# dnbaker/dashing

Hardware: AMD Instinct MI355X
Metric: genome-pairs/sec, all-pairs HLL Jaccard (Ertl-MLE), N=10000 p=14 (higher is better)
Workload: dtype u8/u32 popcount + f64 estimator; 1 GPU; BASELINE configs[2]: 10000 synthetic sketches, p=14 (16384 B each), all-pairs dist on MI355X; n_sketches=10000, p=14, k=31, estimator=ERTL_MLE

## Files before the change

### dashing_amd/csrc/abi.hip

```cpp
#include <algorithm>
#include <cstdlib>
#include <cstring>
#include <new>

#include "ctx.h"

using namespace dsh;

extern "C" {

const char *dsh_backend_name(void) { return "hip:gfx950"; }

int dsh_abi_version(void) { return DSH_ABI_VERSION; }

int dsh_device_count(void)
{
    int n = 0;
    if (hipGetDeviceCount(&n) != hipSuccess) return 0;
    return n;
}

static void release_ctx(dsh_ctx *c)
{
    (void)hipSetDevice(c->device);
// ... 529 lines not shown
        *out = 0;
#endif
    }
    else if (!std::strcmp(name, "npad")) *out = c->lay.Npad;
    else if (!std::strcmp(name, "kpad")) *out = c->Kpad;
    else if (!std::strcmp(name, "cum_bytes")) *out = c->cum_bytes;
    else if (!std::strcmp(name, "sorted")) *out = c->lay.sorted;
    else if (!std::strcmp(name, "ncols")) *out = (int64_t)c->lay.ncols;
    else if (!std::strcmp(name, "lockstep")) *out = c->planes_valid && use_lockstep(c) ? 1 : 0;
    else if (!std::strcmp(name, "tiles")) *out = (int64_t)c->pp.T.size();
    else if (!std::strcmp(name, "bands")) *out = (int64_t)c->last_bands;
    else if (!std::strcmp(name, "items")) *out = (int64_t)c->pp.items.size();
    else if (!std::strcmp(name, "frag_items")) {
        uint64_t f = 0;
        for (uint32_t x : c->pp.band_frags) f += x;
        *out = (int64_t)f;
    }
    else if (!std::strcmp(name, "sparse_items")) *out = (int64_t)c->pp.sp_items.size();
    else if (!std::strcmp(name, "sparse_plane_us")) *out = (int64_t)(c->sparse_ms * 1000.0);
    else if (!std::strcmp(name, "sparse_sided_items")) *out = (int64_t)c->pp.sided_items;
    else if (!std::strcmp(name, "sparse_transposed_items")) *out = (int64_t)c->pp.transposed_items;
    else if (!std::strcmp(name, "sparse_slabs")) *out = (int64_t)c->pp.slabs.size();
    else if (!std::strcmp(name, "sparse_table_slabs")) *out = (int64_t)c->pp.table_slabs;
    else if (!std::strcmp(name, "sparse_planes")) *out = c->sparse_planes;
    else if (!std::strcmp(name, "sparse_sided")) *out = c->sparse_sided;
    else if (!std::strcmp(name, "sparse_cap")) *out = c->sparse_cap;
    else if (!std::strcmp(name, "words_per_plane")) *out = c->W;
    else if (!std::strcmp(name, "avg_tile_planes_x100")) {
        uint64_t tot = 0;
        for (const auto &t : c->pp.T) tot += t.w - t.z;
        *out = c->pp.T.empty() ? 0 : (int64_t)(tot * 100 / c->pp.T.size());
    }
    else return fail(c, DSH_EINVAL, "unknown info %s", name);
    return DSH_OK;
}

}

struct IntOption {
    const char *name;
    int64_t lo, hi;
    const char *range;
    void (*set)(dsh_ctx *c, int64_t v);
};
#define OPT_TO(member, T) [](dsh_ctx *c, int64_t v) { c->member = (T)v; }
static_assert(kGreedyMaxRows == 8192 && plan::kSparseCapMax == 2040, "the ranges below name these");
static const IntOption kIntOptions[] = {
    {"cum_budget_bytes", 1 << 20, INT64_MAX, "too small", OPT_TO(cum_budget, uint64_t)},
    {"knn_square_budget_bytes", 0, INT64_MAX, "must be >= 0", OPT_TO(knn_square_budget, uint64_t)},
    {"threshold_band_bytes", 4, INT64_MAX, "must be at least 4", OPT_TO(threshold_band_bytes, uint64_t)},
    {"pairs_chunk", 1, 1 << 24, "must be in [1, 2^24]", OPT_TO(pairs.chunk, uint64_t)},
    {"cluster_chunk", 1, 1 << 26, "must be in [1, 2^26]", OPT_TO(cc.chunk, uint64_t)},
    {"stats_route", -1, 1, "must be -1 (auto), 0 (dense) or 1 (pairs)", OPT_TO(gs.route, int)},
    {"linkage_route", -1, 1, "must be -1 (auto), 0 (dense) or 1 (pairs)", OPT_TO(lk.route, int)},
    {"linkage_partition", 0, 1, "must be 0 or 1", OPT_TO(lk.partition, int)},
    {"linkage_budget_bytes", 64, INT64_MAX, "must be at least 64", OPT_TO(lk.budget, uint64_t)},
    {"linkage_lds_max", 0, 6144, "must be in [0, 6144]", OPT_TO(lk.lds_max, uint32_t)},
    {"greedy_band_rows", 1, kGreedyMaxRows, "must be in [1, 8192]", OPT_TO(gr.band_rows, uint64_t)},
    {"derive_chunk_bytes", 1, INT64_MAX, "must be at least 1", OPT_TO(derive.chunk_bytes, uint64_t)},
    {"curve_segment", 0, INT64_MAX, "must be >= 0 (0 = the planner's)", OPT_TO(curve.segment, uint64_t)},
    {"curve_scratch_bytes", 1, INT64_MAX, "must be at least 1", OPT_TO(curve.scratch_bytes, uint64_t)},
    {"sort", -1, 1, "must be -1, 0 or 1", OPT_TO(sort_mode, int)},
    {"nsplit", 0, 64, "must be in [0,64]", OPT_TO(nsplit, int)},
    {"part_band_tiles", 1, 1 << 30, "out of range", OPT_TO(part_band_tiles, int)},
    {"xch_tail_bands", 0, 8, "out of range", OPT_TO(tail_bands, int)},
    {"overflow_frag_permille", 0, 1000, "out of range", OPT_TO(overflow_frag_permille, int)},
    {"sparse_planes", -1, 2, "is -1 (auto), 0 (off), 1 or 2", OPT_TO(sparse_planes, int)},
    {"sparse_sided", -1, 1, "is -1 (auto), 0 (off) or 1 (forced)", OPT_TO(sparse_sided, int)},
    {"sparse_lds", 0, 1, "must be 0 or 1", OPT_TO(sparse_lds, int)},
    {"sparse_cap", 0, plan::kSparseCapMax, "must be in [0, 2040]", OPT_TO(sparse_cap, int)},
    {"xch_recv_gate", -1, 1, "is -1 (auto), 0 or 1", OPT_TO(xch.recv_gate, int)},
    {"finalize_signal", -1, 1, "is -1 (auto), 0 or 1", OPT_TO(finalize_signal, int)},
};
#undef OPT_TO

extern "C" int dsh_set_option(dsh_ctx *c, const char *name, int64_t v)
{
    if (!c || !name) return DSH_EINVAL;
    for (const IntOption &o : kIntOptions) {
        if (std::strcmp(name, o.name)) continue;
        if (v < o.lo || v > o.hi) return fail(c, DSH_EINVAL, "%s %s", o.name, o.range);
        o.set(c, v);
        return DSH_OK;
    }
    if (!std::strcmp(name, "kc")) {
        if (v != 0 && v != 16 && v != 32) return fail(c, DSH_EINVAL, "kc must be 0 (auto), 16 or 32");
        c->kc_opt = (int)v;
        c->planes_valid = false;
        return DSH_OK;
    }
    if (!std::strcmp(name, "pair_groups")) {
        if (v != 0 && v != 2 && v != 3) return fail(c, DSH_EINVAL, "pair_groups must be 0 (auto), 2 or 3");
// ... 34 lines not shown
```

### dashing_amd/csrc/ctx.h

```cpp
#pragma once
#include <hip/hip_runtime.h>
#include <rccl/rccl.h>

#include <cstdarg>
#include <cstdio>
#include <cstdlib>
#include <deque>
#include <string>
#include <vector>

#include "../../include/dashing_hip.h"
#include "kernels.h"
#include "plan.h"

struct NoCopy {
    NoCopy() = default;
    NoCopy(const NoCopy &) = delete;
    NoCopy &operator=(const NoCopy &) = delete;
};

struct DevBuf : NoCopy {
    void *ptr = nullptr;
    size_t cap = 0;
    ~DevBuf() { release(); }
// ... 146 lines not shown
    const uint32_t *hk32 = nullptr;
    const uint32_t *hg32 = nullptr;
    const uint32_t *hv32 = nullptr;
    uint32_t pass_sparse_cap = 0;
    bool hk32_valid = false;
    double host_layout_us = 0, host_lists_us = 0, host_keys_wait_us = 0;
    Staging st_perm;
    DevBuf rowoff;
    Staging st_lists;
    uint32_t W = 0, Kpad = 0;
    int emax = 0, elow = 0, cum_bytes = 4;
    int kc = 16;
    int kc_opt = 0;
    int pair_groups = 3;
    int pair_groups_opt = 0;
    int emax_opt = -1;
    int elow_opt = -1;
    int part_band_tiles = 2048;
    int overflow_frag_permille = 500;
    int sparse_planes = -1;
    int sparse_cap = (int)dsh::plan::kSparseCapDefault;
    int sparse_sided = -1;
    int sparse_lds = 1;
    DevBuf sp_tab, sp_lists, sp_len, sp_slabs, sp_items;
    Staging st_sparse;
    std::vector<dsh::plan::U2> sp_have;
    uint64_t sp_serial = 0, lay_serial = 0;
    uint32_t sp_cap_have = 0;
    double sparse_ms = 0;
    std::vector<std::pair<hipEvent_t, hipEvent_t>> ev_sparse;
    int tail_bands = 2;
    std::vector<double> part_ready_ms;
    std::vector<uint64_t> part_floats;
    size_t last_bands = 0;
    uint64_t cum_budget = 8ull << 30;
    int sort_mode = -1;
    int range_sort_min_rows = 1024;
    DevBuf thr_vals;
    uint64_t threshold_band_bytes = (uint64_t)1 << 30;
    uint64_t knn_square_budget = (uint64_t)96 << 30;
    int pair_mfma = 0;
    int finalize_stop = 0;
    int finalize_timing = 0;
    DevBuf phase_cyc;
    int nsplit = 0;
    bool profiling = false;
// ... 258 lines not shown
```

### dashing_amd/csrc/engine.hip

```cpp
#include <algorithm>
#include <chrono>
#include <cstring>

#include "ctx.h"

namespace dsh {

int prepare(dsh_ctx *c, int estim, int want_sorted, bool card_only, uint64_t want_rb, uint64_t want_re, uint32_t nparts,
            int rowsorted, const std::vector<uint64_t> *extra_in)
{
    static const std::vector<uint64_t> kNoExtra;
    std::vector<uint64_t> extra_cached;
    const std::vector<uint64_t> *extra = extra_in ? extra_in : &kNoExtra;
    if (!c->have_sketches) return fail(c, DSH_ESTATE, "no sketches loaded");
    if (estim < 0 || estim > 2) return fail(c, DSH_EINVAL, "bad estimator %d", estim);
    if (want_sorted < 0) {
        want_sorted = c->lay.sorted;
        want_rb = c->lay.rb;
        want_re = c->lay.re;
        rowsorted = 0;
        extra_cached = c->lay.extra;
        extra = &extra_cached;
    }
    if (!want_sorted) rowsorted = 0, extra = &kNoExtra;
// ... 201 lines not shown
{
    JobLayout jl;
    const uint64_t jre = std::min<uint64_t>(job.row_end, c->n);
    const bool full_tri = !job.rect && job.row_begin == 0 && jre >= c->n;
    jl.with_parts = job.nparts > 0 && !job.rect && !job.sorted_rows;
    jl.lre = c->n;
    if (job.sorted_rows) jl.want_sorted = 1;
    else if (!job.rect && jre > job.row_begin &&
             (jl.with_parts || (c->sort_mode != 0 && (full_tri || jre - job.row_begin >= (uint64_t)c->range_sort_min_rows)))) {
        jl.want_sorted = 1;
        jl.lrb = job.row_begin;
        jl.lre = jre;
    }
    jl.with_extra = jl.want_sorted && jl.with_parts && !job.extra.empty() && jl.lre > jl.lrb;
    return jl;
}

constexpr uint64_t kSparseSlabBudget = 2ull << 30;
uint32_t sparse_list_stride(const dsh_ctx *c)
{
    return std::max<uint32_t>(8, (std::min<uint32_t>((uint32_t)c->sparse_cap, plan::kSparseCapMax) + 7) / 8 * 8);
}
int sparse_wordmajor(const dsh_ctx *c) { return c->sparse_lds && c->p <= 15 ? 1 : 0; }
uint64_t sparse_slab_bytes(const dsh_ctx *c)
{
    return ((uint64_t)16 << c->p) + (uint64_t)kTile * sparse_list_stride(c) * sizeof(uint16_t) + kTile * sizeof(uint32_t);
}

plan::Tuning tuning_of(const dsh_ctx *c)
{
    plan::Tuning tu;
    tu.W = c->W;
    tu.kc = c->kc;
    tu.cum_bytes = c->cum_bytes;
    tu.cum_budget = c->cum_budget;
    tu.nsplit = c->nsplit;
    tu.lockstep = use_lockstep(c);
    tu.round_items = 256u * (uint32_t)c->pair_groups;
    tu.small_round_items = c->pair_groups_opt == 0 && c->pair_groups == 3 ? 512u : 0u;
    tu.part_band_tiles = (uint32_t)c->part_band_tiles;
    tu.overflow_frag_max_permille = (uint32_t)c->overflow_frag_permille;
    tu.tail_bands = (uint32_t)c->tail_bands;
    tu.p = c->p;
    tu.sparse_planes = c->sparse_planes;
    tu.sparse_cap = (uint32_t)c->sparse_cap;
    tu.sparse_sided = c->sparse_sided;
// ... 131 lines not shown
        HIPCHK(c, launch_upload(c->stream, c->sp_slabs.ptr, h + ib, sb));
        HIPCHK(c, c->sp_tab.ensure(ns * m * 16));
        HIPCHK(c, c->sp_lists.ensure(ns * kTile * (size_t)cap * sizeof(uint16_t)));
        HIPCHK(c, c->sp_len.ensure(ns * kTile * sizeof(uint32_t)));
        HIPCHK(c, launch_sparse_build(c->stream, (const uint32_t *)c->planes.ptr, L.Npad, c->W, L.ncols, (const uint2 *)c->sp_slabs.ptr,
                                      (uint32_t)ns, cap, sparse_wordmajor(c), (uint32_t *)c->sp_tab.ptr, (uint16_t *)c->sp_lists.ptr, (uint32_t *)c->sp_len.ptr));
        c->sp_have = pp.slabs;
        c->sp_serial = c->lay_serial;
        c->sp_cap_have = cap | (uint32_t)sparse_wordmajor(c) << 31;
        timer.stop(c->prep_ms, true);
    }
    HIPCHK(c, c->st_sparse.sent(c->stream));
    return DSH_OK;
}

int launch_sparse_items(dsh_ctx *c, size_t bi, uint64_t nslots)
{
    const plan::PairPlan &pp = c->pp;
    if (bi >= pp.band_sp_items.size()) return DSH_OK;
    const auto &rg = pp.band_sp_items[bi];
    if (rg.first == rg.second) return DSH_OK;
    hipEvent_t a = c->profiling ? next_event(c) : nullptr, b = c->profiling ? next_event(c) : nullptr;
    if (a && b) (void)hipEventRecord(a, c->stream);
    HIPCHK(c, launch_sparse_count(c->stream, c->cum_bytes, (const uint4 *)c->sp_items.ptr + rg.first, (uint32_t)(rg.second - rg.first),
                                  sparse_wordmajor(c), (const uint32_t *)c->sp_tab.ptr, (const uint16_t *)c->sp_lists.ptr, (const uint32_t *)c->sp_len.ptr,
                                  sparse_list_stride(c), 1u << c->p, c->cum.ptr, nslots));
    if (a && b) {
        (void)hipEventRecord(b, c->stream);
        c->ev_sparse.emplace_back(a, b);
    }
    return DSH_OK;
}

int launch_tile_kernel(dsh_ctx *c, const PairRun &r, size_t bi, uint64_t nslots)
{
    const plan::Layout &L = c->lay;
    const plan::PairPlan &pp = c->pp;
    const uint4 *dt = (const uint4 *)c->tiles.ptr + pp.bands[bi].first;
    const uint4 *di = (const uint4 *)c->items.ptr + r.item_off[bi];
    const uint32_t ni = (uint32_t)(r.item_off[bi + 1] - r.item_off[bi]);
    if (c->pair_mfma)
        HIPCHK(c, launch_pair_counts_mfma(c->stream, c->kc, c->cum_bytes, (const uint32_t *)c->planes.ptr,
                                          L.Npad, c->Kpad, c->W, L.P, dt, di, ni, c->cum.ptr, nslots));
    else if (use_lockstep(c))
        HIPCHK(c, launch_pair_counts_lockstep(c->stream, c->kc, (int)(pp.band_round[bi] / 256), c->cum_bytes, (const uint32_t *)c->planes.ptr,
                                              L.Npad, c->Kpad, c->W, L.P, dt, di, ni, bi < pp.band_frags.size() ? pp.band_frags[bi] : 0u,
                                              c->cum.ptr, nslots));
    else
// ... 131 lines not shown
    q.col_begin = job.col_begin;
    q.col_end = job.col_end;
    r.tu = tuning_of(c);
    if (!plan::build_tiles(c->lay, q, r.tu, pp)) {
        pp.T.clear();
        return DSH_OK;
    }
    c->last_bands = pp.bands.size();
    if ((rc = reserve_lists(c, r))) return rc;
    c->host_lists_us = std::chrono::duration<double, std::micro>(std::chrono::steady_clock::now() - t_l0).count();

    if (jl.with_parts && pp.nparts >= 1 && pp.nparts <= kSigMaxParts && !c->finalize_timing && !c->finalize_stop && c->finalize_signal != 0) {
        r.signal = device_can_wait_value(c);
        if (!r.signal && c->finalize_signal == 1) return fail(c, DSH_ENODEV, "option finalize_signal = 1, but the device does not support hipStreamWaitValue32");
    }
    c->parts_signalled = r.signal;
    if (r.signal && (rc = stage_signal_block(c, r))) return rc;
    if (c->finalize_timing) {
        HIPCHK(c, c->phase_cyc.ensure(16 * sizeof(unsigned long long)));
        HIPCHK(c, hipMemsetAsync(c->phase_cyc.ptr, 0, 16 * sizeof(unsigned long long), c->stream));
    }
    r.fin = finalize_invariants(c, job, jl.with_extra);
    c->ev_sparse.clear();
    if (!pp.sp_items.empty() && (rc = prepare_sparse(c))) return rc;
    for (size_t bi = 0; bi < pp.bands.size(); ++bi) {
        const uint64_t nslots = (uint64_t)(pp.bands[bi].second - pp.bands[bi].first) * kTile * kTile;
        if ((rc = upload_band(c, r, bi))) return rc;
        hipEvent_t a = nullptr, b = nullptr, d = nullptr;
        if (c->profiling) {
            a = next_event(c);
            b = next_event(c);
            d = next_event(c);
            if (a) (void)hipEventRecord(a, c->stream);
        }
        if ((rc = launch_sparse_items(c, bi, nslots))) return rc;
        if ((rc = launch_tile_kernel(c, r, bi, nslots))) return rc;
        if (b) (void)hipEventRecord(b, c->stream);
        if (bi == 0) {
            HIPCHK(c, c->ev_first_tiles.ensure());
            HIPCHK(c, hipEventRecord(c->ev_first_tiles, c->stream));
        }
        r.fin.a.nslots = nslots;
        if ((rc = finalize_band(c, r, bi))) return rc;
        if (d) (void)hipEventRecord(d, c->stream);
        if (a && b && d) {
            r.evp.emplace_back(a, b);
// ... 9 lines not shown
```

### dashing_amd/csrc/host/plan_capi.cpp

```cpp
#include <algorithm>
#include <cstdarg>
#include <cstdio>
#include <cstring>
#include <vector>

#include "../linkage.h"
#include "../mst.h"
#include "../plan.h"
#include "../sketch_plan.h"
#include "../uf.h"

using namespace dsh;
using namespace dsh::plan;

namespace {

struct SparseCheck {
    const uint32_t *gcnt = nullptr;
    int planes = 0;
    uint32_t cap = 0;
    uint32_t *routes = nullptr;
    uint64_t routes_cap = 0;
    const uint32_t *thr = nullptr;
    uint32_t thr_cap = 0;
// ... 725 lines not shown
    sc.planes = sparse_planes;
    sc.cap = sparse_cap;
    sc.thr = thr;
    sc.thr_cap = thr_cap;
    sc.sided = sparse_sided;
    CheckJob job = base_job(n, keys, mode, want_sorted, rb, re, nparts, want_parts, p, cum_budget);
    job.cb = cb, job.ce = ce;
    job.lockstep = lockstep, job.nsplit = nsplit, job.ls_item_chunks = ls_item_chunks;
    job.extra.assign(extra, extra + (extra ? n_extra : 0));
    job.round_items = round_items;
    job.sc = &sc;
    job.resolve();
    if (!job.extra.empty() && !(job.want_sorted && job.mode == 0)) return E.fail("extra segments need a sorted triangle layout");
    Layout L;
    job_layout(job, L);
    Tuning tu;
    PairQuery q;
    PairPlan pp;
    const bool any = job_plan(job, L, tu, q, pp);
    *features = digest_plan(L, tu, q, pp, any, digests);
    return (int)kDigestSections;
}

uint64_t dshh_rowsorted_split(uint64_t n, uint64_t rb, uint64_t re) { return rowsorted_split(n, rb, re); }

int64_t dshh_threshold_bands(uint64_t n, uint64_t rb, uint64_t re, uint64_t ncols, uint64_t band_bytes, uint64_t row_cap,
                             uint64_t *bounds, uint64_t cap)
{
    const uint64_t band_floats = std::max<uint64_t>(band_bytes / sizeof(float), 1);
    if (!ncols && re > n) re = n;
    uint64_t nb = 0;
    if (cap) bounds[0] = rb;
    for (uint64_t b0 = rb; b0 < re;) {
        b0 = ncols ? std::min<uint64_t>(re, b0 + rect_band_rows(ncols, band_floats)) : tri_band_end(n, b0, re, band_floats, row_cap);
        if (++nb >= cap) return -1;
        bounds[nb] = b0;
    }
    return (int64_t)nb;
}

uint64_t dshh_hist_grid(uint64_t units, uint64_t lds_bytes, uint32_t cus, uint64_t *iters)
{
    const uint64_t grid = hist_grid(units, lds_bytes, cus);
    if (iters) *iters = units / (4 * grid) + (units % (4 * grid) ? 1 : 0);
    return grid;
}
// ... 192 lines not shown
```

### dashing_amd/csrc/kernels.h

```cpp
#pragma once
#include <hip/hip_runtime.h>
#include <stdint.h>

#include "consts.h"
#include "sketch_plan.h"

namespace dsh {

hipError_t launch_selfhist_card(hipStream_t st, const uint8_t *regs, uint64_t first, uint64_t n, int p, int estim,
                                int emax, int elow, uint32_t *hist, void *exc, uint8_t *excv, uint32_t *exc_n,
                                uint32_t *keys, uint8_t *tailhist, uint32_t *gcnt, uint32_t *sthr, uint32_t scap);
hipError_t launch_card_from_hist(hipStream_t st, const uint32_t *hist, const uint32_t *keys, uint64_t first, uint64_t n, int p,
                                 int estim, double *card);
inline int colindex_inline(int p, uint32_t E) { return p <= 12 && E <= 256 ? 7 : 3; }
struct ColIndexLaunch {
    const void *exc;
    const uint8_t *excv;
    const uint32_t *exc_n, *keys;
    const double *card;
    const uint8_t *tailhist;
    const uint32_t *perm;
    uint64_t ncols;
    int p;
    uint32_t nblocks, nbuckets, ent_stride, E;
    uint32_t *rec;
    uint32_t *ent;
    uint32_t *nS, *keyS;
    double *cardS;
    uint8_t *thS;
    uint32_t *rl;
};
hipError_t launch_build_colindex(hipStream_t st, const ColIndexLaunch &c);
hipError_t launch_transform(hipStream_t st, const uint8_t *regs, uint64_t n, int p, int vlo,
                            uint32_t P, uint32_t W, uint32_t Npad, uint32_t *planes,
                            const uint32_t *perm);
hipError_t launch_pair_counts(hipStream_t st, int kc, int cum_bytes, const uint32_t *planes,
                              uint32_t Npad, uint32_t Kpad, uint32_t W, uint32_t P,
                              const uint4 *tiles, const uint4 *items, uint32_t nitems, void *cum,
                              uint64_t nslots);

hipError_t launch_sparse_build(hipStream_t st, const uint32_t *planes, uint32_t Npad, uint32_t W, uint64_t ncols, const uint2 *slabs,
                               uint32_t nslabs, uint32_t cap, int wordmajor, uint32_t *tab, uint16_t *lists, uint32_t *len);
hipError_t launch_sparse_count(hipStream_t st, int cum_bytes, const uint4 *items, uint32_t nitems, int wordmajor, const uint32_t *tab,
                               const uint16_t *lists, const uint32_t *len, uint32_t cap, uint32_t m, void *cum, uint64_t nslots);

hipError_t launch_pair_counts_lockstep(hipStream_t st, int kc, int groups, int cum_bytes, const uint32_t *planes,
                                       uint32_t Npad, uint32_t Kpad, uint32_t W, uint32_t P, const uint4 *tiles,
                                       const uint4 *items, uint32_t nitems, uint32_t nfrag, void *cum, uint64_t nslots);
hipError_t launch_pair_counts_mfma(hipStream_t st, int kc, int cum_bytes, const uint32_t *planes,
                                   uint32_t Npad, uint32_t Kpad, uint32_t W, uint32_t P,
                                   const uint4 *tiles, const uint4 *items, uint32_t nitems, void *cum,
                                   uint64_t nslots);

struct FinalizeArgs {
    const void *cum;
    uint64_t nslots;
    const uint4 *tiles;
    const uint32_t *perm;
    const uint64_t *rowoff;
    int hist_bins;
    int pbase;
    int p;
    int estim;
    int result_type;
    double ksinv;
    const uint32_t *nS;
    const uint32_t *keyS;
// ... 219 lines not shown
```

### dashing_amd/csrc/kernels_sparseplane.hip

```cpp
#include <hip/hip_runtime.h>
#include <stdint.h>

#include <algorithm>

#include "kernels.h"
#include "plan.h"

namespace dsh {

namespace {

using plan::kSpItemListA;
using plan::kSpItemTabA;
using plan::kSpItemTransposed;
using plan::kSpPlaneMask;
using plan::kSpSlabA;
using plan::kSpSlabTableOnly;

constexpr int kSpChunk = 16;
constexpr int kSpCounters = 11;

__global__ __launch_bounds__(256) void k_sparse_build(const uint32_t *__restrict__ planes, uint32_t Npad, uint32_t W, uint64_t ncols,
                                                      const uint2 *__restrict__ slabs, uint32_t nslabs, uint32_t cap, int wordmajor,
                                                      uint32_t *__restrict__ tab, uint16_t *__restrict__ lists, uint32_t *__restrict__ len)
{
    const uint32_t lane = threadIdx.x & 63u;
// ... 46 lines not shown
    }
}

__device__ __forceinline__ void csa(uint32_t &h, uint32_t &l, uint32_t a, uint32_t b, uint32_t c)
{
    const uint32_t u = a ^ b;
    h = (a & b) | (u & c);
    l = u ^ c;
}

__device__ __forceinline__ void put32(uint16_t *dst, const uint32_t (&v)[32])
{
#pragma unroll
    for (int q = 0; q < 4; ++q)
        reinterpret_cast<uint4 *>(dst)[q] = make_uint4(v[8 * q] | (v[8 * q + 1] << 16), v[8 * q + 2] | (v[8 * q + 3] << 16),
                                                       v[8 * q + 4] | (v[8 * q + 5] << 16), v[8 * q + 6] | (v[8 * q + 7] << 16));
}
__device__ __forceinline__ void put32(uint32_t *dst, const uint32_t (&v)[32])
{
#pragma unroll
    for (int q = 0; q < 8; ++q) reinterpret_cast<uint4 *>(dst)[q] = make_uint4(v[4 * q], v[4 * q + 1], v[4 * q + 2], v[4 * q + 3]);
}

template <typename CT>
__device__ __forceinline__ void sp_values(uint32_t (&out)[32], const uint32_t (&c)[kSpCounters], uint32_t fl, uint32_t m, uint32_t ll,
                                          const uint32_t *lt)
{
    const bool la = (fl & kSpItemListA) != 0, ta = (fl & kSpItemTabA) != 0;
    const uint32_t kl = !la && !ta ? m - ll : la && !ta ? ll : 0u;
    const uint32_t tsub = !la && !ta ? 0xFFFFFFFFu : 0u, tadd = !la && ta ? 0xFFFFFFFFu : 0u;
    const uint32_t cneg = la != ta ? 0xFFFFFFFFu : 0u;
#pragma unroll
    for (int cc = 0; cc < 32; ++cc) {
        uint32_t cnt = 0;
#pragma unroll
        for (int b = 0; b < kSpCounters; ++b) cnt |= ((c[b] >> cc) & 1u) << b;
        const uint32_t t = lt[cc];
        out[cc] = (kl + (t & tadd) - (t & tsub) + ((cnt ^ cneg) - cneg)) & (sizeof(CT) == 2 ? 0xFFFFu : 0xFFFFFFFFu);
    }
}

template <typename CT>
__device__ __forceinline__ void sp_store_rows(const uint32_t *st, CT *dst, uint32_t tid)
{
    if (sizeof(CT) == 2) {
        const uint32_t at = (tid >> 4) * kTile + (tid & 15u) * 8;
        const uint4 a = *reinterpret_cast<const uint4 *>(st + at), b = *reinterpret_cast<const uint4 *>(st + at + 4);
        *reinterpret_cast<uint4 *>(dst + at) = make_uint4(a.x | (a.y << 16), a.z | (a.w << 16), b.x | (b.y << 16), b.z | (b.w << 16));
    } else {
#pragma unroll
        for (uint32_t h = 0; h < 2; ++h) {
            const uint32_t g = tid + 512 * h, at = (g >> 5) * kTile + (g & 31u) * 4;
            *reinterpret_cast<uint4 *>(dst + at) = *reinterpret_cast<const uint4 *>(st + at);
        }
    }
}

template <typename CT>
__global__ __launch_bounds__(512) void k_sparse_count(const uint4 *__restrict__ items, const uint32_t *__restrict__ tab,
                                                      const uint16_t *__restrict__ lists, const uint32_t *__restrict__ len, uint32_t cap,
                                                      uint32_t m, CT *__restrict__ cum, uint64_t nslots)
// ... 20 lines not shown
#pragma unroll
        for (int q = 0; q < 8; ++q) {
            const bool valid = k0 + q < li;
            const uint32_t pos = valid ? (pw[q >> 1] >> (16 * (q & 1))) & 0xFFFFu : 0u;
            const uint32_t v = tb[(uint64_t)pos * 4];
            x[q] = valid ? v : 0u;
        }
        uint32_t t0, t1, t2, t3, f0, f1, e;
        csa(t0, c[0], c[0], x[0], x[1]);
        csa(t1, c[0], c[0], x[2], x[3]);
        csa(f0, c[1], c[1], t0, t1);
        csa(t2, c[0], c[0], x[4], x[5]);
        csa(t3, c[0], c[0], x[6], x[7]);
        csa(f1, c[1], c[1], t2, t3);
        csa(e, c[2], c[2], f0, f1);
#pragma unroll
        for (int b = 3; b < kSpCounters; ++b) {
            const uint32_t carry = c[b] & e;
            c[b] ^= e;
            e = carry;
        }
    }
    uint32_t out[32];
    sp_values<CT>(out, c, it.y, m, li_all, lenj + w * 32);
    CT *blk = cum + (uint64_t)plane * nslots + (uint64_t)it.x * (kTile * kTile);
    if (!tr) {
        put32(blk + (uint64_t)r * kTile + w * 32, out);
        return;
    }
    for (uint32_t k = 0; k < 4; ++k) {
        if (w == k) {
#pragma unroll
            for (int cc = 0; cc < 32; ++cc) turn[cc * kTile + r] = out[cc];
        }
        __syncthreads();
        sp_store_rows<CT>(turn, blk + (uint64_t)k * 32 * kTile, tid);
        __syncthreads();
    }
}

template <typename CT>
__global__ __launch_bounds__(512) void k_sparse_count_lds(const uint4 *__restrict__ items, uint32_t nitems, const uint32_t *__restrict__ tabw,
                                                          const uint16_t *__restrict__ lists, const uint32_t *__restrict__ len, uint32_t cap,
                                                          uint32_t m, CT *__restrict__ cum, uint64_t nslots)
{
    extern __shared__ __attribute__((aligned(16))) uint32_t sp_lds[];
    const uint32_t g = blockIdx.x, item = (g >> 5) * 8 + (g & 7u), w = (g >> 3) & 3u;
    if (item >= nitems) return;
    const uint4 it = items[item];
    const bool tr = (it.y & kSpItemTransposed) != 0;
    const uint32_t ls = tr ? it.w : it.z, ts = tr ? it.z : it.w, plane = it.y & kSpPlaneMask;
    const uint32_t tid = threadIdx.x, r = tid >> 2, q = tid & 3u;
    const uint32_t lenat = m < 32u * kTile ? 32u * kTile : m;
    const uint4 *src = reinterpret_cast<const uint4 *>(tabw + ((uint64_t)ts * 4 + w) * m);
    for (uint32_t i = tid; i < m / 4; i += 512) reinterpret_cast<uint4 *>(sp_lds)[i] = src[i];
    if (tid < 32) sp_lds[lenat + tid] = len[(uint64_t)ts * kTile + w * 32 + tid];
    __syncthreads();
    const uint32_t li_all = len[(uint64_t)ls * kTile + r];
    const uint32_t li = li_all < cap ? li_all : cap;
    const uint16_t *lp = lists + ((uint64_t)ls * kTile + r) * cap;
    uint32_t c[kSpCounters];
#pragma unroll
    for (int b = 0; b < kSpCounters; ++b) c[b] = 0;
    for (uint32_t k0 = 8 * q; k0 < li; k0 += 32) {
        const uint4 pk = *reinterpret_cast<const uint4 *>(lp + k0);
        const uint32_t pw[4] = {pk.x, pk.y, pk.z, pk.w};
        uint32_t x[8];
#pragma unroll
        for (int j = 0; j < 8; ++j) {
            const bool valid = k0 + j < li;
            const uint32_t pos = valid ? (pw[j >> 1] >> (16 * (j & 1))) & 0xFFFFu : 0u;
            const uint32_t v = sp_lds[pos];
            x[j] = valid ? v : 0u;
        }
        uint32_t t0, t1, t2, t3, f0, f1, e;
        csa(t0, c[0], c[0], x[0], x[1]);
        csa(t1, c[0], c[0], x[2], x[3]);
        csa(f0, c[1], c[1], t0, t1);
        csa(t2, c[0], c[0], x[4], x[5]);
        csa(t3, c[0], c[0], x[6], x[7]);
        csa(f1, c[1], c[1], t2, t3);
        csa(e, c[2], c[2], f0, f1);
#pragma unroll
        for (int b = 3; b < kSpCounters; ++b) {
            const uint32_t carry = c[b] & e;
            c[b] ^= e;
            e = carry;
        }
    }
#pragma unroll
    for (int d = 1; d <= 2; d <<= 1) {
        uint32_t carry = 0;
#pragma unroll
        for (int b = 0; b < kSpCounters; ++b) {
            const uint32_t o = __shfl_xor(c[b], d, 64);
            const uint32_t u = c[b] ^ o;
            const uint32_t sum = u ^ carry;
            carry = (c[b] & o) | (u & carry);
            c[b] = sum;
        }
    }
    CT *blk = cum + (uint64_t)plane * nslots + (uint64_t)it.x * (kTile * kTile);
    if (!tr) {
        if (q != 0) return;
        uint32_t out[32];
        sp_values<CT>(out, c, it.y, m, li_all, sp_lds + lenat);
        put32(blk + (uint64_t)r * kTile + w * 32, out);
        return;
    }
    __syncthreads();
    if (q == 0) {
        uint32_t out[32];
        sp_values<CT>(out, c, it.y, m, li_all, sp_lds + lenat);
#pragma unroll
        for (int cc = 0; cc < 32; ++cc) sp_lds[cc * kTile + r] = out[cc];
    }
    __syncthreads();
    sp_store_rows<CT>(sp_lds, blk + (uint64_t)w * 32 * kTile, tid);
}

}

hipError_t launch_sparse_build(hipStream_t st, const uint32_t *planes, uint32_t Npad, uint32_t W, uint64_t ncols, const uint2 *slabs,
                               uint32_t nslabs, uint32_t cap, int wordmajor, uint32_t *tab, uint16_t *lists, uint32_t *len)
{
    if (nslabs == 0) return hipSuccess;
    if (W < kSpChunk || W % kSpChunk || cap % 8) return hipErrorInvalidValue;
    hipError_t e = hipMemsetAsync(len, 0, (size_t)nslabs * kTile * sizeof(uint32_t), st);
    if (e != hipSuccess) return e;
    const uint64_t units = (uint64_t)nslabs * 2 * (W / kSpChunk);
    hipLaunchKernelGGL(k_sparse_build, dim3((uint32_t)((units + 3) / 4)), dim3(256), 0, st, planes, Npad, W, ncols, slabs, nslabs, cap,
                       wordmajor, tab, lists, len);
    return hipGetLastError();
}

hipError_t launch_sparse_count(hipStream_t st, int cum_bytes, const uint4 *items, uint32_t nitems, int wordmajor, const uint32_t *tab,
                               const uint16_t *lists, const uint32_t *len, uint32_t cap, uint32_t m, void *cum, uint64_t nslots)
{
    if (nitems == 0) return hipSuccess;
    if (cap % 8 || cap > 2047) return hipErrorInvalidValue;
    if (wordmajor) {
        if (m < 512 || m > (1u << 15)) return hipErrorInvalidValue;
        const size_t lds = (size_t)std::max<uint32_t>(m, 32u * kTile) * 4 + 32 * 4;
        const uint32_t grid = (nitems + 7) / 8 * 32;
#define DSH_SPL(CT)                                                                                                                   \
    do {                                                                                                                              \
        const hipError_t e = ensure_dynamic_lds(reinterpret_cast<const void *>(k_sparse_count_lds<CT>), lds);                          \
        if (e != hipSuccess) return e;                                                                                                \
        hipLaunchKernelGGL(k_sparse_count_lds<CT>, dim3(grid), dim3(512), lds, st, items, nitems, tab, lists, len, cap, m, (CT *)cum, nslots); \
    } while (0)
        if (cum_bytes == 2) DSH_SPL(uint16_t);
        else DSH_SPL(uint32_t);
#undef DSH_SPL
        return hipGetLastError();
    }
    if (cum_bytes == 2)
        hipLaunchKernelGGL(k_sparse_count<uint16_t>, dim3(nitems), dim3(512), 0, st, items, tab, lists, len, cap, m, (uint16_t *)cum, nslots);
    else
        hipLaunchKernelGGL(k_sparse_count<uint32_t>, dim3(nitems), dim3(512), 0, st, items, tab, lists, len, cap, m, (uint32_t *)cum, nslots);
    return hipGetLastError();
}

hipError_t preload_sparseplane_kernels()
{
    hipFuncAttributes fa;
    return hipFuncGetAttributes(&fa, reinterpret_cast<const void *>(k_sparse_build));
}

}
```

### dashing_amd/csrc/plan.cpp

```cpp
#include "plan.h"

#include <algorithm>
#include <cstring>

namespace dsh {
namespace plan {

uint64_t tri_index(uint64_t n, uint64_t i, uint64_t j) { return i * (2 * n - i - 1) / 2 + j - (i + 1); }

uint64_t tri_span(uint64_t n, uint64_t rb, uint64_t re)
{
    if (re > n) re = n;
    if (rb >= re) return 0;
    const uint64_t cnt = re - rb;
    return cnt * (n - 1) - (rb + re - 1) * cnt / 2;
}

uint64_t tri_band_end(uint64_t n, uint64_t b0, uint64_t re, uint64_t band_floats, uint64_t row_cap)
{
    const uint64_t max_rows = std::min<uint64_t>(std::max<uint64_t>(row_cap, 1), kBandMaxRows);
    uint64_t b1 = b0, span = 0;
    do {
        span += n - 1 - b1;
        ++b1;
// ... 851 lines not shown
    std::vector<uint32_t> xcd_of(NT, 0);
    size_t load[nx] = {0};
    for (uint32_t b : cols) {
        size_t x = 0;
        for (size_t y = 1; y < nx; ++y)
            if (load[y] < load[x]) x = y;
        xcd_of[b] = (uint32_t)x;
        load[x] += per_col[b];
    }
    std::vector<U4> lists[nx];
    for (size_t k = first; k < last; ++k) lists[xcd_of[table_block(sp_items[k])]].push_back(sp_items[k]);
    for (auto &l : lists)
        std::stable_sort(l.begin(), l.end(), [&](const U4 &a, const U4 &b) {
            const U4 &ta = T[bd.first + a.x], &tb = T[bd.first + b.x];
            const uint32_t ca = table_block(a), cb = table_block(b), pa = a.y & kSpPlaneMask, pb = b.y & kSpPlaneMask;
            return ca != cb ? ca < cb : pa != pb ? pa > pb : ta.x + ta.y < tb.x + tb.y;
        });
    size_t q = first;
    for (size_t r = 0; q < last; ++r)
        for (size_t x = 0; x < nx; ++x)
            if (r < lists[x].size()) sp_items[q++] = lists[x][r];
}

static void route_sparse(const Layout &L, const Tuning &tu, const SparseGate &gate, PairPlan &pp)
{
    const std::vector<U4> &T = pp.T;
    const uint32_t NT = L.Npad / kTile;
    pp.sp.assign(T.size(), 0);
    pp.spb.assign(T.size(), 0);
    pp.sided_items = pp.transposed_items = pp.table_slabs = 0;
    pp.band_sp_items.assign(pp.bands.size(), std::make_pair((size_t)0, (size_t)0));
    if (!gate.any()) return;
    pp.slab_of.assign((size_t)NT * std::max<uint32_t>(L.P, 1), -1);
    std::vector<uint8_t> listed;
    auto slab = [&](uint32_t b, uint32_t pl, bool lists) -> uint32_t {
        int32_t &s = pp.slab_of[(size_t)b * L.P + pl];
        if (s < 0) {
            s = (int32_t)pp.slabs.size();
            pp.slabs.push_back(U2{b, pl | (gate.sided_can && sided_polarity(L, b, L.pbase + 1 + (int)pl) ? kSpSlabA : 0u)});
            listed.push_back(0);
        }
        if (lists) listed[(size_t)s] = 1;
        return (uint32_t)s;
    };
    for (size_t bi = 0; bi < pp.bands.size(); ++bi) {
        const auto &bd = pp.bands[bi];
// ... 352 lines not shown
```

### dashing_amd/csrc/plan.h

```cpp
#pragma once
#include <stddef.h>
#include <stdint.h>

#include <algorithm>
#include <utility>
#include <vector>

#include "consts.h"

namespace dsh {
namespace plan {

struct U4 { uint32_t x, y, z, w; };
struct U2 { uint32_t x, y; };

inline int key_lo(uint32_t k) { return (int)(k & 63u); }
inline int key_L(uint32_t k) { return (int)((k >> 6) & 63u); }
inline int key_T(uint32_t k) { return (int)((k >> 12) & 63u); }
inline int key_hi(uint32_t k) { return (int)((k >> 18) & 63u); }
inline bool key_bad(uint32_t k) { return (k & 0x80000000u) != 0; }

uint64_t tri_index(uint64_t n, uint64_t i, uint64_t j);
uint64_t tri_span(uint64_t n, uint64_t rb, uint64_t re);
void partition_rows(uint64_t n, uint32_t nparts, uint32_t align, uint64_t *bounds);
// ... 84 lines not shown
    pe = std::max(pb, std::max(T_i, T_j) - pbase);
}
inline void tile_planes(const Layout &L, uint32_t ti, uint32_t tj, int &pb, int &pe)
{
    tile_planes(L.blk_lo[ti], L.blk_L[ti], L.blk_T[ti], L.blk_lo[tj], L.blk_L[tj], L.blk_T[tj], L.pbase, pb, pe);
}

void shard_bounds(const Layout &L, uint32_t nshards, std::vector<uint32_t> &tb);
inline uint64_t shard_row(const std::vector<uint32_t> &tb, uint32_t r, uint64_t n) { return std::min<uint64_t>(n, (uint64_t)tb[r] * kTile); }

struct PairQuery {
    int rect = 0;
    int sorted_rows = 0;
    int want_parts = 0;
    uint64_t row_begin = 0, row_end = 0, col_begin = 0, col_end = 0;
};

constexpr uint32_t kSparseCapDefault = 1280, kSparseCapMax = 2040;
constexpr int kSparseAutoPlanes = 2;
constexpr bool kSparseSidedAuto = true;
constexpr uint32_t kSpPlaneMask = 0xFFu;
constexpr uint32_t kSpItemListA = 1u << 8, kSpItemTabA = 1u << 9, kSpItemTransposed = 1u << 10;
constexpr uint32_t kSpSlabA = 1u << 8, kSpSlabTableOnly = 1u << 9;

struct Tuning {
    uint32_t W = 0;
    int kc = 32;
    int cum_bytes = 2;
    uint64_t cum_budget = 8ull << 30;
    int nsplit = 0;
    bool lockstep = true;
    int ls_item_chunks = 64;
    uint32_t part_band_tiles = 2048;
    uint32_t round_items = 512;
    uint32_t small_round_items = 0;
    uint32_t overflow_frag_max_permille = 500;
    uint32_t tail_bands = 2;
    uint32_t tail_permille = 100;
    uint32_t tail_permille2 = 350;
    uint32_t tail_head_min_rounds = 7;
    int sparse_planes = 0;
    uint32_t sparse_cap = kSparseCapDefault;
    uint32_t sparse_max_slabs = 1u << 16;
    int sparse_sided = 0;
    int p = 0;
};
// ... 46 lines not shown
```

Baseline: 4.420 billion pairs/s.

## Process runs of sparse items per block, reusing LDS-resident table across items

The word-major sparse count kernel now loops over a run of items (default 4) per block, reloading the table into LDS only when the table slab changes. Each quad lane now computes and stores 8 output columns directly instead of lane 0 computing all 32. The transposed-output staging buffer is resized by counter type. This is meant to cut repeated global-to-LDS table fills and launch overhead, at the cost of fewer blocks and serialized items within a block. It also adds an info counter for table fills and a debug cut path behind a compile flag.

```diff
diff --git a/dashing_amd/csrc/abi.hip b/dashing_amd/csrc/abi.hip
--- a/dashing_amd/csrc/abi.hip
+++ b/dashing_amd/csrc/abi.hip
@@ -575,6 +575,13 @@
     else if (!std::strcmp(name, "sparse_transposed_items")) *out = (int64_t)c->pp.transposed_items;
     else if (!std::strcmp(name, "sparse_slabs")) *out = (int64_t)c->pp.slabs.size();
     else if (!std::strcmp(name, "sparse_table_slabs")) *out = (int64_t)c->pp.table_slabs;
+    else if (!std::strcmp(name, "sparse_table_fills")) {
+        uint64_t f = 0;
+        if (c->sparse_run_used)
+            for (const auto &rg : c->pp.band_sp_items) f += plan::sparse_table_fills(c->pp.sp_items.data() + rg.first, rg.second - rg.first, c->sparse_run_used);
+        *out = (int64_t)f;
+    }
+    else if (!std::strcmp(name, "sparse_run")) *out = c->sparse_run > 0 ? c->sparse_run : (int64_t)plan::kSparseRunDefault;
     else if (!std::strcmp(name, "sparse_planes")) *out = c->sparse_planes;
     else if (!std::strcmp(name, "sparse_sided")) *out = c->sparse_sided;
     else if (!std::strcmp(name, "sparse_cap")) *out = c->sparse_cap;
@@ -597,7 +604,7 @@
     void (*set)(dsh_ctx *c, int64_t v);
 };
 #define OPT_TO(member, T) [](dsh_ctx *c, int64_t v) { c->member = (T)v; }
-static_assert(kGreedyMaxRows == 8192 && plan::kSparseCapMax == 2040, "the ranges below name these");
+static_assert(kGreedyMaxRows == 8192 && plan::kSparseCapMax == 2040 && plan::kSparseRunMax == 65536, "the ranges below name these");
 static const IntOption kIntOptions[] = {
     {"cum_budget_bytes", 1 << 20, INT64_MAX, "too small", OPT_TO(cum_budget, uint64_t)},
     {"knn_square_budget_bytes", 0, INT64_MAX, "must be >= 0", OPT_TO(knn_square_budget, uint64_t)},
@@ -621,6 +628,7 @@
     {"sparse_planes", -1, 2, "is -1 (auto), 0 (off), 1 or 2", OPT_TO(sparse_planes, int)},
     {"sparse_sided", -1, 1, "is -1 (auto), 0 (off) or 1 (forced)", OPT_TO(sparse_sided, int)},
     {"sparse_lds", 0, 1, "must be 0 or 1", OPT_TO(sparse_lds, int)},
+    {"sparse_run", 0, plan::kSparseRunMax, "must be in [0, 65536]", OPT_TO(sparse_run, int)},
     {"sparse_cap", 0, plan::kSparseCapMax, "must be in [0, 2040]", OPT_TO(sparse_cap, int)},
     {"xch_recv_gate", -1, 1, "is -1 (auto), 0 or 1", OPT_TO(xch.recv_gate, int)},
     {"finalize_signal", -1, 1, "is -1 (auto), 0 or 1", OPT_TO(finalize_signal, int)},
diff --git a/dashing_amd/csrc/ctx.h b/dashing_amd/csrc/ctx.h
--- a/dashing_amd/csrc/ctx.h
+++ b/dashing_amd/csrc/ctx.h
@@ -192,6 +192,8 @@
     int sparse_cap = (int)dsh::plan::kSparseCapDefault;
     int sparse_sided = -1;
     int sparse_lds = 1;
+    int sparse_run = 0;
+    uint32_t sparse_run_used = 0;
     DevBuf sp_tab, sp_lists, sp_len, sp_slabs, sp_items;
     Staging st_sparse;
     std::vector<dsh::plan::U2> sp_have;
diff --git a/dashing_amd/csrc/engine.hip b/dashing_amd/csrc/engine.hip
--- a/dashing_amd/csrc/engine.hip
+++ b/dashing_amd/csrc/engine.hip
@@ -247,6 +247,7 @@
     return std::max<uint32_t>(8, (std::min<uint32_t>((uint32_t)c->sparse_cap, plan::kSparseCapMax) + 7) / 8 * 8);
 }
 int sparse_wordmajor(const dsh_ctx *c) { return c->sparse_lds && c->p <= 15 ? 1 : 0; }
+uint32_t sparse_run_of(const dsh_ctx *c) { return c->sparse_run > 0 ? (uint32_t)c->sparse_run : plan::kSparseRunDefault; }
 uint64_t sparse_slab_bytes(const dsh_ctx *c)
 {
     return ((uint64_t)16 << c->p) + (uint64_t)kTile * sparse_list_stride(c) * sizeof(uint16_t) + kTile * sizeof(uint32_t);
@@ -424,8 +425,9 @@
     if (rg.first == rg.second) return DSH_OK;
     hipEvent_t a = c->profiling ? next_event(c) : nullptr, b = c->profiling ? next_event(c) : nullptr;
     if (a && b) (void)hipEventRecord(a, c->stream);
+    if (sparse_wordmajor(c)) c->sparse_run_used = sparse_run_of(c);
     HIPCHK(c, launch_sparse_count(c->stream, c->cum_bytes, (const uint4 *)c->sp_items.ptr + rg.first, (uint32_t)(rg.second - rg.first),
-                                  sparse_wordmajor(c), (const uint32_t *)c->sp_tab.ptr, (const uint16_t *)c->sp_lists.ptr, (const uint32_t *)c->sp_len.ptr,
+                                  sparse_run_of(c), sparse_wordmajor(c), (const uint32_t *)c->sp_tab.ptr, (const uint16_t *)c->sp_lists.ptr, (const uint32_t *)c->sp_len.ptr,
                                   sparse_list_stride(c), 1u << c->p, c->cum.ptr, nslots));
     if (a && b) {
         (void)hipEventRecord(b, c->stream);
@@ -603,6 +605,7 @@
     }
     r.fin = finalize_invariants(c, job, jl.with_extra);
     c->ev_sparse.clear();
+    c->sparse_run_used = 0;
     if (!pp.sp_items.empty() && (rc = prepare_sparse(c))) return rc;
     for (size_t bi = 0; bi < pp.bands.size(); ++bi) {
         const uint64_t nslots = (uint64_t)(pp.bands[bi].second - pp.bands[bi].first) * kTile * kTile;
diff --git a/dashing_amd/csrc/host/plan_capi.cpp b/dashing_amd/csrc/host/plan_capi.cpp
--- a/dashing_amd/csrc/host/plan_capi.cpp
+++ b/dashing_amd/csrc/host/plan_capi.cpp
@@ -771,6 +771,12 @@
     return (int)kDigestSections;
 }
 
+uint64_t dshh_sparse_table_fills(const uint32_t *items4, uint64_t n, uint32_t run)
+{
+    static_assert(sizeof(U4) == 4 * sizeof(uint32_t), "an item is four words");
+    return sparse_table_fills(reinterpret_cast<const U4 *>(items4), (size_t)n, run);
+}
+
 uint64_t dshh_rowsorted_split(uint64_t n, uint64_t rb, uint64_t re) { return rowsorted_split(n, rb, re); }
 
 int64_t dshh_threshold_bands(uint64_t n, uint64_t rb, uint64_t re, uint64_t ncols, uint64_t band_bytes, uint64_t row_cap,
diff --git a/dashing_amd/csrc/kernels.h b/dashing_amd/csrc/kernels.h
--- a/dashing_amd/csrc/kernels.h
+++ b/dashing_amd/csrc/kernels.h
@@ -41,8 +41,9 @@
 
 hipError_t launch_sparse_build(hipStream_t st, const uint32_t *planes, uint32_t Npad, uint32_t W, uint64_t ncols, const uint2 *slabs,
                                uint32_t nslabs, uint32_t cap, int wordmajor, uint32_t *tab, uint16_t *lists, uint32_t *len);
-hipError_t launch_sparse_count(hipStream_t st, int cum_bytes, const uint4 *items, uint32_t nitems, int wordmajor, const uint32_t *tab,
-                               const uint16_t *lists, const uint32_t *len, uint32_t cap, uint32_t m, void *cum, uint64_t nslots);
+hipError_t launch_sparse_count(hipStream_t st, int cum_bytes, const uint4 *items, uint32_t nitems, uint32_t run, int wordmajor,
+                               const uint32_t *tab, const uint16_t *lists, const uint32_t *len, uint32_t cap, uint32_t m, void *cum,
+                               uint64_t nslots);
 
 hipError_t launch_pair_counts_lockstep(hipStream_t st, int kc, int groups, int cum_bytes, const uint32_t *planes,
                                        uint32_t Npad, uint32_t Kpad, uint32_t W, uint32_t P, const uint4 *tiles,
diff --git a/dashing_amd/csrc/kernels_sparseplane.hip b/dashing_amd/csrc/kernels_sparseplane.hip
--- a/dashing_amd/csrc/kernels_sparseplane.hip
+++ b/dashing_amd/csrc/kernels_sparseplane.hip
@@ -2,6 +2,7 @@
 #include <stdint.h>
 
 #include <algorithm>
+#include <cstdlib>
 
 #include "kernels.h"
 #include "plan.h"
@@ -94,21 +95,24 @@
     for (int q = 0; q < 8; ++q) reinterpret_cast<uint4 *>(dst)[q] = make_uint4(v[4 * q], v[4 * q + 1], v[4 * q + 2], v[4 * q + 3]);
 }
 
-template <typename CT>
-__device__ __forceinline__ void sp_values(uint32_t (&out)[32], const uint32_t (&c)[kSpCounters], uint32_t fl, uint32_t m, uint32_t ll,
-                                          const uint32_t *lt)
+template <typename CT, int N>
+__device__ __forceinline__ void sp_values(uint32_t (&out)[N], const uint32_t (&c)[kSpCounters], uint32_t c0, uint32_t fl, uint32_t m,
+                                          uint32_t ll, const uint32_t *lt)
 {
     const bool la = (fl & kSpItemListA) != 0, ta = (fl & kSpItemTabA) != 0;
     const uint32_t kl = !la && !ta ? m - ll : la && !ta ? ll : 0u;
     const uint32_t tsub = !la && !ta ? 0xFFFFFFFFu : 0u, tadd = !la && ta ? 0xFFFFFFFFu : 0u;
     const uint32_t cneg = la != ta ? 0xFFFFFFFFu : 0u;
-#pragma unroll
-    for (int cc = 0; cc < 32; ++cc) {
+    uint32_t cs[kSpCounters];
+#pragma unroll
+    for (int b = 0; b < kSpCounters; ++b) cs[b] = c[b] >> c0;
+#pragma unroll
+    for (int j = 0; j < N; ++j) {
         uint32_t cnt = 0;
 #pragma unroll
-        for (int b = 0; b < kSpCounters; ++b) cnt |= ((c[b] >> cc) & 1u) << b;
-        const uint32_t t = lt[cc];
-        out[cc] = (kl + (t & tadd) - (t & tsub) + ((cnt ^ cneg) - cneg)) & (sizeof(CT) == 2 ? 0xFFFFu : 0xFFFFFFFFu);
+        for (int b = 0; b < kSpCounters; ++b) cnt |= ((cs[b] >> j) & 1u) << b;
+        const uint32_t t = lt[j];
+        out[j] = (kl + (t & tadd) - (t & tsub) + ((cnt ^ cneg) - cneg)) & (sizeof(CT) == 2 ? 0xFFFFu : 0xFFFFFFFFu);
     }
 }
 
@@ -175,7 +179,7 @@
         }
     }
     uint32_t out[32];
-    sp_values<CT>(out, c, it.y, m, li_all, lenj + w * 32);
+    sp_values<CT, 32>(out, c, 0u, it.y, m, li_all, lenj + w * 32);
     CT *blk = cum + (uint64_t)plane * nslots + (uint64_t)it.x * (kTile * kTile);
     if (!tr) {
         put32(blk + (uint64_t)r * kTile + w * 32, out);
@@ -192,84 +196,122 @@
     }
 }
 
+__device__ __forceinline__ void put8(uint16_t *dst, const uint32_t (&v)[8])
+{
+    *reinterpret_cast<uint4 *>(dst) = make_uint4(v[0] | (v[1] << 16), v[2] | (v[3] << 16), v[4] | (v[5] << 16), v[6] | (v[7] << 16));
+}
+__device__ __forceinline__ void put8(uint32_t *dst, const uint32_t (&v)[8])
+{
+    reinterpret_cast<uint4 *>(dst)[0] = make_uint4(v[0], v[1], v[2], v[3]);
+    reinterpret_cast<uint4 *>(dst)[1] = make_uint4(v[4], v[5], v[6], v[7]);
+}
+
+template <bool kPartial>
+__device__ __forceinline__ void sp_step_lds(uint32_t (&c)[kSpCounters], const uint32_t *tabl, const uint4 pk, uint32_t left)
+{
+    const uint32_t pw[4] = {pk.x, pk.y, pk.z, pk.w};
+    uint32_t x[8];
+#pragma unroll
+    for (int j = 0; j < 8; ++j) {
+        const bool valid = !kPartial || (uint32_t)j < left;
+        const uint32_t pos = valid ? (pw[j >> 1] >> (16 * (j & 1))) & 0xFFFFu : 0u;
+        const uint32_t v = tabl[pos];
+        x[j] = valid ? v : 0u;
+    }
+    uint32_t t0, t1, t2, t3, f0, f1, e;
+    csa(t0, c[0], c[0], x[0], x[1]);
+    csa(t1, c[0], c[0], x[2], x[3]);
+    csa(f0, c[1], c[1], t0, t1);
+    csa(t2, c[0], c[0], x[4], x[5]);
+    csa(t3, c[0], c[0], x[6], x[7]);
+    csa(f1, c[1], c[1], t2, t3);
+    csa(e, c[2], c[2], f0, f1);
+#pragma unroll
+    for (int b = 3; b < kSpCounters; ++b) {
+        const uint32_t carry = c[b] & e;
+        c[b] ^= e;
+        e = carry;
+    }
+}
+
 template <typename CT>
-__global__ __launch_bounds__(512) void k_sparse_count_lds(const uint4 *__restrict__ items, uint32_t nitems, const uint32_t *__restrict__ tabw,
-                                                          const uint16_t *__restrict__ lists, const uint32_t *__restrict__ len, uint32_t cap,
-                                                          uint32_t m, CT *__restrict__ cum, uint64_t nslots)
+__global__ __launch_bounds__(512) void k_sparse_count_lds(const uint4 *__restrict__ items, uint32_t nitems, uint32_t run,
+                                                          const uint32_t *__restrict__ tabw, const uint16_t *__restrict__ lists,
+                                                          const uint32_t *__restrict__ len, uint32_t cap, uint32_t m, CT *__restrict__ cum,
+                                                          uint64_t nslots, uint32_t stop)
 {
     extern __shared__ __attribute__((aligned(16))) uint32_t sp_lds[];
-    const uint32_t g = blockIdx.x, item = (g >> 5) * 8 + (g & 7u), w = (g >> 3) & 3u;
-    if (item >= nitems) return;
-    const uint4 it = items[item];
-    const bool tr = (it.y & kSpItemTransposed) != 0;
-    const uint32_t ls = tr ? it.w : it.z, ts = tr ? it.z : it.w, plane = it.y & kSpPlaneMask;
-    const uint32_t tid = threadIdx.x, r = tid >> 2, q = tid & 3u;
-    const uint32_t lenat = m < 32u * kTile ? 32u * kTile : m;
-    const uint4 *src = reinterpret_cast<const uint4 *>(tabw + ((uint64_t)ts * 4 + w) * m);
-    for (uint32_t i = tid; i < m / 4; i += 512) reinterpret_cast<uint4 *>(sp_lds)[i] = src[i];
-    if (tid < 32) sp_lds[lenat + tid] = len[(uint64_t)ts * kTile + w * 32 + tid];
-    __syncthreads();
-    const uint32_t li_all = len[(uint64_t)ls * kTile + r];
-    const uint32_t li = li_all < cap ? li_all : cap;
-    const uint16_t *lp = lists + ((uint64_t)ls * kTile + r) * cap;
-    uint32_t c[kSpCounters];
-#pragma unroll
-    for (int b = 0; b < kSpCounters; ++b) c[b] = 0;
-    for (uint32_t k0 = 8 * q; k0 < li; k0 += 32) {
-        const uint4 pk = *reinterpret_cast<const uint4 *>(lp + k0);
-        const uint32_t pw[4] = {pk.x, pk.y, pk.z, pk.w};
-        uint32_t x[8];
-#pragma unroll
-        for (int j = 0; j < 8; ++j) {
-            const bool valid = k0 + j < li;
-            const uint32_t pos = valid ? (pw[j >> 1] >> (16 * (j & 1))) & 0xFFFFu : 0u;
-            const uint32_t v = sp_lds[pos];
-            x[j] = valid ? v : 0u;
-        }
-        uint32_t t0, t1, t2, t3, f0, f1, e;
-        csa(t0, c[0], c[0], x[0], x[1]);
-        csa(t1, c[0], c[0], x[2], x[3]);
-        csa(f0, c[1], c[1], t0, t1);
-        csa(t2, c[0], c[0], x[4], x[5]);
-        csa(t3, c[0], c[0], x[6], x[7]);
-        csa(f1, c[1], c[1], t2, t3);
-        csa(e, c[2], c[2], f0, f1);
-#pragma unroll
-        for (int b = 3; b < kSpCounters; ++b) {
-            const uint32_t carry = c[b] & e;
-            c[b] ^= e;
-            e = carry;
-        }
-    }
-#pragma unroll
-    for (int d = 1; d <= 2; d <<= 1) {
-        uint32_t carry = 0;
-#pragma unroll
-        for (int b = 0; b < kSpCounters; ++b) {
-            const uint32_t o = __shfl_xor(c[b], d, 64);
-            const uint32_t u = c[b] ^ o;
-            const uint32_t sum = u ^ carry;
-            carry = (c[b] & o) | (u & carry);
-            c[b] = sum;
-        }
-    }
-    CT *blk = cum + (uint64_t)plane * nslots + (uint64_t)it.x * (kTile * kTile);
-    if (!tr) {
-        if (q != 0) return;
-        uint32_t out[32];
-        sp_values<CT>(out, c, it.y, m, li_all, sp_lds + lenat);
-        put32(blk + (uint64_t)r * kTile + w * 32, out);
-        return;
-    }
-    __syncthreads();
-    if (q == 0) {
-        uint32_t out[32];
-        sp_values<CT>(out, c, it.y, m, li_all, sp_lds + lenat);
-#pragma unroll
-        for (int cc = 0; cc < 32; ++cc) sp_lds[cc * kTile + r] = out[cc];
-    }
-    __syncthreads();
-    sp_store_rows<CT>(sp_lds, blk + (uint64_t)w * 32 * kTile, tid);
+#ifdef DSH_SPARSE_CUT
+    const uint32_t cut = stop;
+#else
+    constexpr uint32_t cut = 0;
+#endif
+    CT *turn = reinterpret_cast<CT *>(sp_lds + m);
+    const uint32_t g = blockIdx.x, x = g & 7u, w = (g >> 3) & 3u, first = (g >> 5) * run;
+    const uint32_t tid = threadIdx.x, r = tid >> 2, q = tid & 3u, c0 = 8 * q;
+    uint32_t have = 0xFFFFFFFFu;
+    uint32_t lt[8];
+    for (uint32_t i = 0; i < run; ++i) {
+        const uint32_t item = x + 8 * (first + i);
+        if (item >= nitems) break;
+        const uint4 it = items[item];
+        const bool tr = (it.y & kSpItemTransposed) != 0;
+        const uint32_t ls = tr ? it.w : it.z, ts = tr ? it.z : it.w, plane = it.y & kSpPlaneMask;
+        if (ts != have) {
+            if (i) __syncthreads();
+            const uint4 *src = reinterpret_cast<const uint4 *>(tabw + ((uint64_t)ts * 4 + w) * m);
+            for (uint32_t k = tid; k < m / 4; k += 512) reinterpret_cast<uint4 *>(sp_lds)[k] = src[k];
+            const uint4 *lq = reinterpret_cast<const uint4 *>(len + (uint64_t)ts * kTile + w * 32 + c0);
+            const uint4 l0 = lq[0], l1 = lq[1];
+            lt[0] = l0.x, lt[1] = l0.y, lt[2] = l0.z, lt[3] = l0.w, lt[4] = l1.x, lt[5] = l1.y, lt[6] = l1.z, lt[7] = l1.w;
+            __syncthreads();
+            have = ts;
+        }
+        if (cut == 1) continue;
+        const uint32_t li_all = len[(uint64_t)ls * kTile + r];
+        const uint32_t li = li_all < cap ? li_all : cap;
+        const uint16_t *lp = lists + ((uint64_t)ls * kTile + r) * cap;
+        uint32_t c[kSpCounters];
+#pragma unroll
+        for (int b = 0; b < kSpCounters; ++b) c[b] = 0;
+        uint32_t k0 = 8 * q;
+        for (; k0 + 8 <= li; k0 += 32) sp_step_lds<false>(c, sp_lds, *reinterpret_cast<const uint4 *>(lp + k0), 8);
+        if (k0 < li) sp_step_lds<true>(c, sp_lds, *reinterpret_cast<const uint4 *>(lp + k0), li - k0);
+        if (cut == 2) continue;
+#pragma unroll
+        for (int d = 1; d <= 2; d <<= 1) {
+            uint32_t carry = 0;
+#pragma unroll
+            for (int b = 0; b < kSpCounters; ++b) {
+                const uint32_t o = __shfl_xor(c[b], d, 64);
+                const uint32_t u = c[b] ^ o;
+                const uint32_t sum = u ^ carry;
+                carry = (c[b] & o) | (u & carry);
+                c[b] = sum;
+            }
+        }
+        if (cut == 3) {
+            uint32_t all = 0xFFFFFFFFu;
+#pragma unroll
+            for (int b = 0; b < kSpCounters; ++b) all &= c[b];
+            if (all == 0xFFFFFFFFu && cap == 1) turn[tid] = (CT)all;
+            continue;
+        }
+        uint32_t out[8];
+        sp_values<CT, 8>(out, c, c0, it.y, m, li_all, lt);
+        CT *blk = cum + (uint64_t)plane * nslots + (uint64_t)it.x * (kTile * kTile);
+        if (!tr) {
+            put8(blk + (uint64_t)r * kTile + w * 32 + c0, out);
+            continue;
+        }
+        __syncthreads();
+#pragma unroll
+        for (int j = 0; j < 8; ++j) turn[(c0 + j) * kTile + r] = (CT)out[j];
+        __syncthreads();
+        const uint4 *ts4 = reinterpret_cast<const uint4 *>(turn);
+        uint4 *dst = reinterpret_cast<uint4 *>(blk + (uint64_t)w * 32 * kTile);
+        for (uint32_t k = tid; k < 32 * kTile * sizeof(CT) / 16; k += 512) dst[k] = ts4[k];
+    }
 }
 
 }
@@ -287,20 +329,28 @@
     return hipGetLastError();
 }
 
-hipError_t launch_sparse_count(hipStream_t st, int cum_bytes, const uint4 *items, uint32_t nitems, int wordmajor, const uint32_t *tab,
-                               const uint16_t *lists, const uint32_t *len, uint32_t cap, uint32_t m, void *cum, uint64_t nslots)
+hipError_t launch_sparse_count(hipStream_t st, int cum_bytes, const uint4 *items, uint32_t nitems, uint32_t run, int wordmajor,
+                               const uint32_t *tab, const uint16_t *lists, const uint32_t *len, uint32_t cap, uint32_t m, void *cum,
+                               uint64_t nslots)
 {
     if (nitems == 0) return hipSuccess;
-    if (cap % 8 || cap > 2047) return hipErrorInvalidValue;
+    if (cap % 8 || cap > 2047 || run == 0) return hipErrorInvalidValue;
     if (wordmajor) {
         if (m < 512 || m > (1u << 15)) return hipErrorInvalidValue;
-        const size_t lds = (size_t)std::max<uint32_t>(m, 32u * kTile) * 4 + 32 * 4;
-        const uint32_t grid = (nitems + 7) / 8 * 32;
+        const uint32_t per_x = (nitems + 7) / 8;
+        run = std::min(run, per_x);
+        const uint32_t grid = (per_x + run - 1) / run * 32;
+        uint32_t stop = 0;
+#ifdef DSH_SPARSE_CUT
+        if (const char *s = std::getenv("DSH_SPARSE_STOP")) stop = (uint32_t)std::atoi(s);
+#endif
 #define DSH_SPL(CT)                                                                                                                   \
     do {                                                                                                                              \
+        const size_t lds = (size_t)m * 4 + 32 * kTile * sizeof(CT);                                                                   \
         const hipError_t e = ensure_dynamic_lds(reinterpret_cast<const void *>(k_sparse_count_lds<CT>), lds);                          \
         if (e != hipSuccess) return e;                                                                                                \
-        hipLaunchKernelGGL(k_sparse_count_lds<CT>, dim3(grid), dim3(512), lds, st, items, nitems, tab, lists, len, cap, m, (CT *)cum, nslots); \
+        hipLaunchKernelGGL(k_sparse_count_lds<CT>, dim3(grid), dim3(512), lds, st, items, nitems, run, tab, lists, len, cap, m,        \
+                           (CT *)cum, nslots, stop);                                                                                  \
     } while (0)
         if (cum_bytes == 2) DSH_SPL(uint16_t);
         else DSH_SPL(uint32_t);
diff --git a/dashing_amd/csrc/plan.cpp b/dashing_amd/csrc/plan.cpp
--- a/dashing_amd/csrc/plan.cpp
+++ b/dashing_amd/csrc/plan.cpp
@@ -897,6 +897,22 @@
             if (r < lists[x].size()) sp_items[q++] = lists[x][r];
 }
 
+uint64_t sparse_table_fills(const U4 *items, size_t n, uint32_t run)
+{
+    if (run == 0) return 0;
+    uint64_t fills = 0;
+    for (size_t x = 0; x < 8 && x < n; ++x) {
+        uint32_t have = 0;
+        size_t i = 0;
+        for (size_t k = x; k < n; k += 8, i = i + 1 == run ? 0 : i + 1) {
+            const uint32_t ts = items[k].y & kSpItemTransposed ? items[k].z : items[k].w;
+            if (i == 0 || ts != have) fills += 4;
+            have = ts;
+        }
+    }
+    return fills;
+}
+
 static void route_sparse(const Layout &L, const Tuning &tu, const SparseGate &gate, PairPlan &pp)
 {
     const std::vector<U4> &T = pp.T;
diff --git a/dashing_amd/csrc/plan.h b/dashing_amd/csrc/plan.h
--- a/dashing_amd/csrc/plan.h
+++ b/dashing_amd/csrc/plan.h
@@ -130,6 +130,8 @@
 constexpr uint32_t kSpPlaneMask = 0xFFu;
 constexpr uint32_t kSpItemListA = 1u << 8, kSpItemTabA = 1u << 9, kSpItemTransposed = 1u << 10;
 constexpr uint32_t kSpSlabA = 1u << 8, kSpSlabTableOnly = 1u << 9;
+constexpr uint32_t kSparseRunDefault = 4, kSparseRunMax = 1u << 16;
+uint64_t sparse_table_fills(const U4 *items, size_t n, uint32_t run);
 
 struct Tuning {
     uint32_t W = 0;
```

Result: faster. 4.606 billion pairs/s (median of 6 runs) (+4.2%).
